# netapp-rickhuang-ai/spark-rapids-ml-nai

Measured on AMD Instinct MI355X. Metric: fit-time speedup vs Spark-ML CPU (geomean over reference headline workloads, 1Mx3000 fp32), higher is better.
Workload: dtype fp32

## Files before the change

spark_rapids_ml_nai_amd/ops/__init__.py:

```python
from __future__ import annotations

import math
import os
from typing import Any, Dict, Iterator, Optional, Tuple

import numpy as np
import torch

from . import native
from ..utils.determinism import deterministic

__all__ = ["col_moments", "gram", "xw", "dgemm", "sign_flip", "is_native", "xtv", "row_sqnorm",
           "logreg_binary_loss_grad", "nearest_centroid", "cluster_sums", "csr_logreg_binary_loss_grad",
           "csr_spmm", "csr_spmtm", "csr_col_moments", "logistic_loss_grad"]


def is_native(t: torch.Tensor) -> bool:
    return t.is_cuda


def _c(t: torch.Tensor) -> torch.Tensor:
    return t if t.is_contiguous() else t.contiguous()


# ... 427 lines not shown


def certify_tau16(n: int) -> float:
    return 1.01 * (2.0 * F16_U + F16_U * F16_U + 1.01 * float(n) * 2.0 ** -24)


def f16_radius_terms(n: int, scale: float, tau: float) -> Tuple[float, float, float]:
    a = F16_A / scale
    z = 2.02 * a * math.sqrt(n) * (1.0 + F16_U)
    z2 = 2.02 * float(n) * a * a
    wmax = math.sqrt(n) * 32768.0 / scale
    return (z + 2.0 ** -24 * wmax) / (2.0 * tau), z, z2


class F16Planes:

    def __init__(self, X: torch.Tensor, mu: torch.Tensor) -> None:
        m, n = X.shape
        self.X, self.m, self.n = X, m, n
        self.mu = _c(mu.float().view(-1))
        dev = X.device
        st = native.stream(dev)
        self.xnorm = torch.empty(m, dtype=torch.float32, device=dev)
        amax = zeros(1, dtype=torch.int32, device=dev)
        native.call("srml_row_sqnorm_centered_amax_f32", X.data_ptr(), m, n, X.stride(0), self.mu.data_ptr(),
                    self.xnorm.data_ptr(), amax.data_ptr(), st)
        a = float(amax.view(torch.float32).item())
        self.ok = math.isfinite(a) and a > 0.0
        self.scale = 1.0
        self.P = None
        if not self.ok:
            return
        e = math.frexp(a)[1] - 1
        if not -100 <= 13 - e <= 100:
            self.ok = False
            return
        self.scale = 2.0 ** (13 - e)
        self.kp = (n + 15) // 16 * 16
        self.rows_pad = max(256, (m + 255) // 256 * 256)
        self.P = torch.empty((self.rows_pad // 256, self.kp // 16, 256, 16), dtype=torch.float16, device=dev)
        self.ovf = zeros(1, dtype=torch.int32, device=dev)
        native.call("srml_split_f16_tiled_centered", X.data_ptr(), m, n, X.stride(0), self.mu.data_ptr(), self.kp,
                    self.rows_pad, self.scale, self.P.data_ptr(), self.ovf.data_ptr(), st)
        self.tau = certify_tau16(n)
        self.xadd, self.z, self.z2 = f16_radius_terms(n, self.scale, self.tau)


F16_CAND_CAP = 64


def _f16_centre_planes(F: F16Planes, C: torch.Tensor, approx: bool) -> Tuple[torch.Tensor, ...]:
    k, dev = C.shape[0], F.X.device
    st = native.stream(dev)
    Cd = _c(C.to(dev)) if C.dtype in (torch.float32, torch.float64) else _c(C.to(dev, torch.float32))
    crows = max(256, (k + 255) // 256 * 256)
    W = torch.empty((k, F.n), dtype=torch.float32, device=dev)
    cn = torch.empty(crows, dtype=torch.float32, device=dev)
    cg = torch.empty(k, dtype=torch.float32, device=dev)
    zero2 = torch.empty(2, dtype=torch.int32, device=dev)
    native.call("srml_f16_centre_prep", Cd.data_ptr(), int(Cd.dtype == torch.float64), k, F.n, F.mu.data_ptr(),
                float(2.0 * F.tau), int(bool(approx)), W.data_ptr(), cn.data_ptr(), cg.data_ptr(), zero2.data_ptr(), st)
    CP = torch.empty((crows // 256, F.kp // 16, 256, 16), dtype=torch.float16, device=dev)
    native.call("srml_split_f16_tiled_centered", W.data_ptr(), k, F.n, W.stride(0), None, F.kp, crows, F.scale,
                CP.data_ptr(), zero2[0:1].data_ptr(), st)
    return W, cn, cg, zero2, CP, crows


def nearest_f16_labels(F: F16Planes, C: torch.Tensor) -> Optional[torch.Tensor]:
    if F.kp != 128 or os.environ.get("SRML_F16_ROWLOOP", "1") == "0":
        return None
    dev = F.X.device
    _, cn, _, _, CP, crows = _f16_centre_planes(F, C, True)
    labels = torch.empty(F.m, dtype=torch.int32, device=dev)
    rc = native.lib().srml_nearest_f16_rowloop(F.P.data_ptr(), F.m, F.rows_pad, F.kp, CP.data_ptr(), C.shape[0],
                                                crows, cn.data_ptr(), float(-2.0 / (F.scale * F.scale)),
                                                labels.data_ptr(), native.stream(dev))
    if rc == -2:
        return None
    if rc != 0:
        raise RuntimeError("srml_nearest_f16_rowloop failed (%d)" % rc)
    return labels


def nearest_centroid_f16(F: F16Planes, C: torch.Tensor, approx: bool = False) -> Tuple[torch.Tensor, torch.Tensor]:
    m, k, dev = F.m, C.shape[0], F.X.device
    st = native.stream(dev)
    W, cn, cg, zero2, CP, crows = _f16_centre_planes(F, C, approx)
    ovf = zero2[0:1]
    xadd, z, z2 = (0.0, 0.0, 0.0) if approx else (F.xadd, F.z, F.z2)
    dscale = -2.0 / (F.scale * F.scale)
    nslot = int(native.lib().srml_nearest_centroid_f16_top2_nslot(k))
    labels = torch.empty(m, dtype=torch.int32, device=dev)
    dist = torch.empty(m, dtype=torch.float32, device=dev)
    flagged = torch.empty(m, dtype=torch.int32, device=dev)
    thr = torch.empty(m, dtype=torch.float32, device=dev)
    cnt = zero2[1:2]
    step = split_rows_per_launch(k)
    for r0 in range(0, m, step):
        mc = min(step, m - r0)
        keys = torch.empty(mc * nslot, dtype=torch.int64, device=dev)
        lob = torch.empty(mc * nslot, dtype=torch.float32, device=dev)
        Pc = F.P[r0 // 256: (r0 + mc + 255) // 256]
        xn = F.xnorm[r0: r0 + mc]
        native.call("srml_nearest_centroid_f16_top2", Pc.data_ptr(), mc, Pc.shape[0] * 256, F.kp, CP.data_ptr(), k,
                    crows, cn.data_ptr(), cg.data_ptr(), xn.data_ptr(), dscale, xadd, keys.data_ptr(), lob.data_ptr(),
                    st)
        c0 = int(cnt.item()) if r0 else 0
        native.call("srml_split_top2_select_f16_thr", keys.data_ptr(), lob.data_ptr(), mc, nslot, xn.data_ptr(),
                    cg.data_ptr(), xadd, z, z2, ovf.data_ptr(), labels[r0:].data_ptr(), dist[r0:].data_ptr(),
                    flagged.data_ptr(), cnt.data_ptr(), thr.data_ptr(), st)
        if r0:
            nc = int(cnt.item())
            flagged[c0:nc] += r0
        del keys, lob
    nf = int(cnt.item())
    _CERTIFY_STATS["rows"] += m
    _CERTIFY_STATS["refined"] += nf
    if nf:
        rows = flagged[:nf]
        X = F.X
        assert X.stride(1) == 1
        cap = F16_CAND_CAP
        cand = torch.empty(nf * cap, dtype=torch.int32, device=dev)
        stepr = split_rows_per_launch(k)
        plane = F.P is not None and os.environ.get("SRML_F16_GATHER", "plane") == "plane"
        ccount = torch.empty(nf, dtype=torch.int32, device=dev) if plane else zeros(nf, dtype=torch.int32,
                                                                                          device=dev)
        scratch = None if plane else zeros(1, dtype=torch.int32, device=dev)
        for q0 in range(0, nf, stepr):
            nq = min(stepr, nf - q0)
            rq = rows[q0: q0 + nq]
            rp = max(256, (nq + 255) // 256 * 256)
            Pr = torch.empty((rp // 256, F.kp // 16, 256, 16), dtype=torch.float16, device=dev)
            if plane:
                xr = torch.empty(nq, dtype=torch.float32, device=dev)
                native.call("srml_f16_plane_gather_rows_ex", F.P.data_ptr(), F.rows_pad, F.kp, rq.data_ptr(), nq, rp,
                            Pr.data_ptr(), F.xnorm.data_ptr(), xr.data_ptr(), ccount[q0:].data_ptr(), st)
            else:
                native.call("srml_split_f16_tiled_centered_rows", X.data_ptr(), X.stride(0), rq.data_ptr(), nq, F.n,
                            F.mu.data_ptr(), F.kp, rp, F.scale, Pr.data_ptr(), scratch.data_ptr(), st)
                xr = F.xnorm.index_select(0, rq.long())
            native.call("srml_nearest_centroid_f16_cand", Pr.data_ptr(), nq, rp, F.kp, CP.data_ptr(), k, crows,
                        cn.data_ptr(), cg.data_ptr(), xr.data_ptr(), dscale, xadd, thr[q0:].data_ptr(),
                        ccount[q0:].data_ptr(), cand[q0 * cap:].data_ptr(), cap, st)
            del Pr
        native.call("srml_kmeans_cand_exact", X.data_ptr(), X.stride(0), F.mu.data_ptr(), W.data_ptr(), W.stride(0),
                    F.n, k, rows.data_ptr(), nf, ccount.data_ptr(), cand.data_ptr(), cap, labels.data_ptr(),
                    dist.data_ptr(), st)
    return labels, dist


def quantizer_planes(X: torch.Tensor) -> Optional[F16Planes]:
    if not X.is_cuda or X.dtype != torch.float32 or X.dim() != 2 or X.shape[1] < 16 or X.stride(1) != 1:
        return None
    mu = col_moments(X, need_sq=False)[0].div_(max(X.shape[0], 1)).float()
    F = F16Planes(X, mu)
    return F if F.ok else None


def nearest_list(X: torch.Tensor, C: torch.Tensor, F: Optional[F16Planes] = None,
                 xnorm: Optional[torch.Tensor] = None) -> torch.Tensor:
    if F is not None and C.shape[0] > 256:
        lab = nearest_f16_labels(F, C)
        return lab if lab is not None else nearest_centroid_f16(F, C, approx=True)[0]
    return nearest_centroid(X, C, xnorm)[0]


def split_rows_per_launch(k: int) -> int:
    ct = max(1, (int(k) + 255) // 256)
    return max(256, (0xFFFFFFFF // 512 // ct) * 256)


def kmeans_filter_mode() -> str:
    v = os.environ.get("SRML_KMEANS_FILTER", "f16").lower()
    if v not in ("f16", "bf16"):
        raise ValueError("SRML_KMEANS_FILTER must be f16 or bf16, got %r" % v)
    return v


def nearest_centroid_split(XP: torch.Tensor, m: int, C: torch.Tensor, xnorm: torch.Tensor,
                           cnorm: Optional[torch.Tensor] = None, approx: bool = False,
                           X: Optional[torch.Tensor] = None, mu: Optional[torch.Tensor] = None
                           ) -> Tuple[torch.Tensor, torch.Tensor]:
    k = C.shape[0]
    Cf = C.float()
    if mu is not None:
        Cf = Cf - mu.float().view(1, -1).to(Cf.device)
        cnorm = None
    if cnorm is None:
# ... 2056 lines not shown
```

spark_rapids_ml_nai_amd/ops/csrc/splitmm.hip:

```cpp
#include "common.h"

#include "tile.h"
#include <stdlib.h>

namespace {
using srml_tile::orderable;
using srml_tile::unorderable;

typedef short bf16x8 __attribute__((ext_vector_type(8)));
typedef _Float16 halfx8 __attribute__((ext_vector_type(8)));
typedef unsigned uintx4 __attribute__((ext_vector_type(4)));
typedef unsigned uintx2 __attribute__((ext_vector_type(2)));

__device__ __forceinline__ unsigned bf16_rn(float f) {
  unsigned u = __float_as_uint(f);
  u += 0x7fffu + ((u >> 16) & 1u);
  return u >> 16;
}
__device__ __forceinline__ float bf16_f(unsigned b) { return __uint_as_float(b << 16); }

__global__ __launch_bounds__(256) void split_kernel(const float* __restrict__ X, long m, int n, long ld, int kp,
                                                    long rows_pad, unsigned short* __restrict__ P) {
  const int q4 = kp >> 2;
  const long total = rows_pad * q4;
  const long plane = rows_pad * (long)kp;
  for (long i = (long)blockIdx.x * 256 + threadIdx.x; i < total; i += (long)gridDim.x * 256) {
    const long r = i / q4;
    const int c = (int)(i - r * q4) * 4;
    unsigned h[4], md[4], lo[4];
#pragma unroll
    for (int j = 0; j < 4; ++j) {
      const float x = (r < m && c + j < n) ? X[r * ld + c + j] : 0.f;
      h[j] = bf16_rn(x);
      const float r1 = x - bf16_f(h[j]);
      md[j] = bf16_rn(r1);
      lo[j] = bf16_rn(r1 - bf16_f(md[j]));
    }
    const long o = r * kp + c;
    *reinterpret_cast<uintx2*>(P + o) = uintx2{h[0] | (h[1] << 16), h[2] | (h[3] << 16)};
    *reinterpret_cast<uintx2*>(P + plane + o) = uintx2{md[0] | (md[1] << 16), md[2] | (md[3] << 16)};
    *reinterpret_cast<uintx2*>(P + 2 * plane + o) = uintx2{lo[0] | (lo[1] << 16), lo[2] | (lo[3] << 16)};
  }
}

__global__ __launch_bounds__(256) void split_tiled_kernel(const float* __restrict__ X, long m, int n, long ld, int kp,
                                                          long rows_pad, unsigned short* __restrict__ P,
                                                          const float* __restrict__ mu,
                                                          const int* __restrict__ ridx = nullptr) {
  const int ks_n = kp >> 4;
  const long total = rows_pad * ks_n;
  const long plane = rows_pad * (long)kp;
  const bool vec = (ld & 3) == 0 && (reinterpret_cast<uintptr_t>(X) & 15) == 0;
  for (long i = (long)blockIdx.x * 256 + threadIdx.x; i < total; i += (long)gridDim.x * 256) {
    const long img = i >> 8;
    const int rr = (int)(i & 255);
    const long tile = img / ks_n;
    const int c0 = (int)(img - tile * ks_n) * 16;
    const long r = tile * 256 + rr;
    const long rs = ridx && r < m ? (long)ridx[r] : r;
    float x[16];
    if (vec && r < m && c0 + 16 <= n) {
#pragma unroll
      for (int q = 0; q < 4; ++q) {
        const floatx4 v = *reinterpret_cast<const floatx4*>(X + rs * ld + c0 + 4 * q);
        x[4 * q] = v[0]; x[4 * q + 1] = v[1]; x[4 * q + 2] = v[2]; x[4 * q + 3] = v[3];
      }
    } else {
#pragma unroll
      for (int j = 0; j < 16; ++j) x[j] = (r < m && c0 + j < n) ? X[rs * ld + c0 + j] : 0.f;
    }
    if (mu && r < m) {
#pragma unroll
      for (int j = 0; j < 16; ++j)
        if (c0 + j < n) x[j] -= mu[c0 + j];
    }
    unsigned hw[8], mw[8], lw[8];
#pragma unroll
    for (int j = 0; j < 16; j += 2) {
      unsigned h2[2], m2[2], l2[2];
#pragma unroll
      for (int u = 0; u < 2; ++u) {
        h2[u] = bf16_rn(x[j + u]);
        const float r1 = x[j + u] - bf16_f(h2[u]);
        m2[u] = bf16_rn(r1);
        l2[u] = bf16_rn(r1 - bf16_f(m2[u]));
      }
// ... 317 lines not shown
#pragma unroll
      for (int r = 0; r < 16; ++r) acc[a][b][r] = 0.f;

  auto mma_step = [&](int cur) {
    bf16x8 fb[3][TN];
#pragma unroll
    for (int p = 0; p < 3; ++p)
#pragma unroll
      for (int nt = 0; nt < TN; ++nt)
        fb[p][nt] = *reinterpret_cast<const bf16x8*>(&st[cur].B[p][wn * (BN / WN) + nt * 32 + li][8 * lk]);
#pragma unroll
    for (int mt = 0; mt < TM; ++mt) {
      bf16x8 fa[3];
#pragma unroll
      for (int p = 0; p < 3; ++p)
        fa[p] = *reinterpret_cast<const bf16x8*>(&st[cur].A[p][wm * (BM / WM) + mt * 32 + li][8 * lk]);
#pragma unroll
      for (int nt = 0; nt < TN; ++nt) {
        acc[mt][nt] = __builtin_amdgcn_mfma_f32_32x32x16_bf16(fa[2], fb[0][nt], acc[mt][nt], 0, 0, 0);
        acc[mt][nt] = __builtin_amdgcn_mfma_f32_32x32x16_bf16(fa[1], fb[1][nt], acc[mt][nt], 0, 0, 0);
        acc[mt][nt] = __builtin_amdgcn_mfma_f32_32x32x16_bf16(fa[0], fb[2][nt], acc[mt][nt], 0, 0, 0);
        acc[mt][nt] = __builtin_amdgcn_mfma_f32_32x32x16_bf16(fa[1], fb[0][nt], acc[mt][nt], 0, 0, 0);
        acc[mt][nt] = __builtin_amdgcn_mfma_f32_32x32x16_bf16(fa[0], fb[1][nt], acc[mt][nt], 0, 0, 0);
        acc[mt][nt] = __builtin_amdgcn_mfma_f32_32x32x16_bf16(fa[0], fb[0][nt], acc[mt][nt], 0, 0, 0);
      }
    }
  };
  auto gload = [&](int kt, uintx4 (&a)[3], uintx4 (&b)[3]) {
    const long ko = (long)kt * SBK;
#pragma unroll
    for (int p = 0; p < 3; ++p) {
      a[p] = *reinterpret_cast<const uintx4*>(xa + p * xplane + ko);
      b[p] = *reinterpret_cast<const uintx4*>(ca + p * cplane + ko);
    }
  };
  auto lstore = [&](int stage, const uintx4 (&a)[3], const uintx4 (&b)[3]) {
#pragma unroll
    for (int p = 0; p < 3; ++p) {
      *reinterpret_cast<uintx4*>(&st[stage].A[p][sr][sh]) = a[p];
      *reinterpret_cast<uintx4*>(&st[stage].B[p][sr][sh]) = b[p];
    }
  };
  const int nk = kp / SBK;
  if (PF == 1) {
    uintx4 ra[3], rb[3];
    gload(0, ra, rb);
    lstore(0, ra, rb);
    __syncthreads();
    int cur = 0;
    for (int kt = 0; kt < nk; ++kt) {
      const bool more = kt + 1 < nk;
      if (more) gload(kt + 1, ra, rb);
      mma_step(cur);
      if (more) lstore(cur ^ 1, ra, rb);
      __syncthreads();
      cur ^= 1;
    }
  } else {
    uintx4 ra0[3], rb0[3], ra1[3], rb1[3];
    gload(0, ra0, rb0);
    if (nk > 1) gload(1, ra1, rb1);
    lstore(0, ra0, rb0);
    __syncthreads();
    int kt = 0;
    for (; kt + 2 <= nk; kt += 2) {
      if (kt + 2 < nk) gload(kt + 2, ra0, rb0);
      mma_step(0);
      lstore(1, ra1, rb1);
      __syncthreads();
      if (kt + 3 < nk) gload(kt + 3, ra1, rb1);
      mma_step(1);
      if (kt + 2 < nk) lstore(0, ra0, rb0);
      __syncthreads();
    }
    if (kt < nk) mma_step(0);
  }

  split_epilogue<BM, BN, WM, WN>(acc, row0, col0, m, k, cnorm, best, wm, wn, li, lk);
}

typedef __attribute__((address_space(3))) void* lds_vptr;
typedef __attribute__((address_space(1))) void* gbl_vptr;

template <bool TILED, int NP = 6, bool TOP2 = false, int WN_ = 4, bool PRIO = false, bool CAND = false, int RING = 0>
__global__ __launch_bounds__(WN_ * 128, WN_ == 4 ? 1 : 2) void nearest_centroid_split_glds_kernel(
    const unsigned short* __restrict__ XP, long m, long xrows, int kp, const unsigned short* __restrict__ CP, int k,
    long crows, const float* __restrict__ cnorm, unsigned long long* __restrict__ best, int n_ctiles,
    float* __restrict__ lob = nullptr, const float* __restrict__ cg = nullptr, const float* __restrict__ xnorm = nullptr,
    float dscale = -2.f, float xadd = 0.f, const float* __restrict__ thr = nullptr, int* __restrict__ ccount = nullptr,
    int* __restrict__ cand = nullptr, int cap = 0) {
  static_assert(!CAND || (NP == 1 && TOP2), "candidate lists come from the fp16 filter");
  static_assert(WN_ == 4 || (WN_ == 2 && NP != 6), "256 x 128 tiles are built for the filter passes");
  static_assert(NP == 6 || NP == 3 || (NP == 1 && TOP2), "NP = 1 is the fp16 certified filter");
  constexpr int BM = 256, WM = 2, WN = WN_, BN = 64 * WN, TM = 4, TN = 2;
  constexpr int NPL = NP == 6 ? 3 : (NP == 3 ? 2 : 1);
  constexpr int XCH = NPL * (BM / 32), CCH = NPL * (BN / 32);
  constexpr int CPW = (XCH + CCH) / (WM * WN);
  static_assert((XCH + CCH) % (WM * WN) == 0, "chunks split evenly over the waves");
  constexpr int KPB = RING ? RING / 10 : NP == 1 ? 3 : (NP == 3 && WN_ == 4 ? 2 : 1);
  constexpr int NG = RING ? RING % 10 : NP == 1 && WN_ == 4 ? 3 : 2;
  static_assert(!RING || (NP == 1 && KPB >= 1 && NG >= 2), "ring override is for the fp16 filter");
  constexpr int NS = (KPB > 1 || RING) ? NG * KPB : 3;
  constexpr int STAGE = NPL * (BM + BN) * 16;
  __shared__ __attribute__((aligned(1024))) unsigned short lds[NS][STAGE];
  const int bid = xcd_remap(blockIdx.x, gridDim.x);
  const long rtile = bid / n_ctiles;
  const int ctile = bid % n_ctiles;
  const long row0 = rtile * BM;
  const int col0 = ctile * BN;
  const int t = threadIdx.x;
  const int lane = t & 63, wid = t >> 6;
  const int wm = wid / WN, wn = wid % WN;
  const int li = lane & 31, lk = lane >> 5;
  const long xplane = xrows * (long)kp, cplane = crows * (long)kp;

  const unsigned short* src[CPW];
  int dst_off[CPW];
#pragma unroll
  for (int i = 0; i < CPW; ++i) {
    const int c = wid * CPW + i;
    const bool isx = c < XCH;
    const int q = isx ? c / (BM / 32) : (c - XCH) / (BN / 32);
    const int j = isx ? c % (BM / 32) : (c - XCH) % (BN / 32);
    const int r = 32 * j + (lane >> 1);
    const int lh = (lane & 1) ^ ((lane >> 4) & 1);
    if (TILED) {
      const int ks_n = kp / SBK;
      if (isx) src[i] = XP + q * xplane + ((rtile * ks_n) << 12) + 512 * j + lane * 8;
      else src[i] = CP + q * cplane + (((long)(col0 >> 8) * ks_n) << 12) + 16 * (col0 & 255) + 512 * j + lane * 8;
    } else if (isx) {
      long xr = row0 + r;
      if (xr >= xrows) xr = xrows - 1;
      src[i] = XP + q * xplane + xr * kp + 8 * lh;
    } else {
      src[i] = CP + q * cplane + (long)(col0 + r) * kp + 8 * lh;
    }
    dst_off[i] = isx ? (q * BM + 32 * j) * 16 : (NPL * BM + q * BN + 32 * j) * 16;
  }
  auto issue = [&](int kt, int stage) {
    unsigned short* base = &lds[stage][0];
#pragma unroll
    for (int i = 0; i < CPW; ++i) {
      __builtin_amdgcn_global_load_lds((gbl_vptr)(src[i] + (TILED ? ((long)kt << 12) : (long)kt * SBK)),
                                       (lds_vptr)(base + dst_off[i]), 16, 0, 0);
    }
  };

  floatx16 acc[TM][TN];
#pragma unroll
  for (int a = 0; a < TM; ++a)
#pragma unroll
    for (int b = 0; b < TN; ++b)
#pragma unroll
      for (int r = 0; r < 16; ++r) acc[a][b][r] = 0.f;

  const int ph = lk ^ ((li >> 3) & 1);
  const int nk = kp / SBK;
  auto compute = [&](int st) {
    bf16x8 fb[NPL][TN];
#pragma unroll
    for (int p = 0; p < NPL; ++p)
#pragma unroll
      for (int nt = 0; nt < TN; ++nt)
        fb[p][nt] = *reinterpret_cast<const bf16x8*>(
            &lds[st][(NPL * BM + p * BN + wn * (BN / WN) + nt * 32 + li) * 16 + 8 * ph]);
#pragma unroll
    for (int mt = 0; mt < TM; ++mt) {
      bf16x8 fa[NPL];
#pragma unroll
      for (int p = 0; p < NPL; ++p)
        fa[p] = *reinterpret_cast<const bf16x8*>(&lds[st][(p * BM + wm * (BM / WM) + mt * 32 + li) * 16 + 8 * ph]);
#pragma unroll
      for (int nt = 0; nt < TN; ++nt) {
        if constexpr (NP == 1) {
          acc[mt][nt] = __builtin_amdgcn_mfma_f32_32x32x16_f16(__builtin_bit_cast(halfx8, fb[0][nt]),
                                                               __builtin_bit_cast(halfx8, fa[0]), acc[mt][nt], 0,
                                                               0, 0);
        } else {
          if constexpr (NP == 6) {
            acc[mt][nt] = __builtin_amdgcn_mfma_f32_32x32x16_bf16(fa[2], fb[0][nt], acc[mt][nt], 0, 0, 0);
            acc[mt][nt] = __builtin_amdgcn_mfma_f32_32x32x16_bf16(fa[1], fb[1][nt], acc[mt][nt], 0, 0, 0);
            acc[mt][nt] = __builtin_amdgcn_mfma_f32_32x32x16_bf16(fa[0], fb[2][nt], acc[mt][nt], 0, 0, 0);
          }
          acc[mt][nt] = __builtin_amdgcn_mfma_f32_32x32x16_bf16(fa[1], fb[0][nt], acc[mt][nt], 0, 0, 0);
          acc[mt][nt] = __builtin_amdgcn_mfma_f32_32x32x16_bf16(fa[0], fb[1][nt], acc[mt][nt], 0, 0, 0);
          acc[mt][nt] = __builtin_amdgcn_mfma_f32_32x32x16_bf16(fa[0], fb[0][nt], acc[mt][nt], 0, 0, 0);
        }
      }
    }
  };
  if constexpr (KPB == 1 && !RING) {
    static_assert(CPW == 6, "the counted wait below leaves one step (CPW loads) in flight");
    issue(0, 0);
    if (nk > 1) issue(1, 1);
    int stage = 0;
    for (int kt = 0; kt < nk; ++kt) {
      if (kt + 1 < nk) asm volatile("s_waitcnt vmcnt(6)" ::: "memory");
      else asm volatile("s_waitcnt vmcnt(0)" ::: "memory");
      __builtin_amdgcn_s_barrier();
      if (kt + 2 < nk) issue(kt + 2, stage == 0 ? 2 : stage - 1);
      if (PRIO) __builtin_amdgcn_s_setprio(1);
      compute(stage);
      if (PRIO) __builtin_amdgcn_s_setprio(0);
      stage = stage == 2 ? 0 : stage + 1;
    }
  } else {
#pragma unroll
    for (int j = 0; j < (NG - 1) * KPB; ++j)
      if (j < nk) issue(j, j);
    for (int kt = 0; kt < nk; kt += KPB) {
      if (NG >= 3 && kt + (NG - 1) * KPB <= nk)
        asm volatile("s_waitcnt vmcnt(%0)" ::"i"((NG - 2) * KPB * CPW) : "memory");
      else asm volatile("s_waitcnt vmcnt(0)" ::: "memory");
      __builtin_amdgcn_s_barrier();
#pragma unroll
      for (int j = 0; j < KPB; ++j)
        if (kt + (NG - 1) * KPB + j < nk) issue(kt + (NG - 1) * KPB + j, (kt + (NG - 1) * KPB + j) % NS);
      if (PRIO) __builtin_amdgcn_s_setprio(1);
#pragma unroll
      for (int j = 0; j < KPB; ++j)
        if (kt + j < nk) compute((kt + j) % NS);
      if (PRIO) __builtin_amdgcn_s_setprio(0);
    }
  }
  if (CAND)
    split_epilogue_cand_t<BM, BN, WM, WN>(acc, row0, col0, m, k, cnorm, cg, xnorm, wm, wn, li, lk, dscale, xadd, thr,
                                          ccount, cand, cap);
  else if (TOP2 && NP == 1)
    split_epilogue_top2_t<BM, BN, WM, WN>(acc, row0, col0, ctile, m, k, cnorm, cg, xnorm, best, lob, n_ctiles * WN, wm,
                                          wn, li, lk, dscale, xadd);
  else if (TOP2)
    split_epilogue_top2<BM, BN, WM, WN>(acc, row0, col0, ctile, m, k, cnorm, cg, xnorm, best, lob, n_ctiles * WN, wm,
                                        wn, li, lk, dscale, xadd);
  else
    split_epilogue<BM, BN, WM, WN>(acc, row0, col0, m, k, cnorm, best, wm, wn, li, lk);
}

__global__ __launch_bounds__(256) void split_top2_select_kernel(const unsigned long long* __restrict__ keys,
                                                                const float* __restrict__ lob, long m, int nslot,
                                                                const float* __restrict__ xnorm,
                                                                const float* __restrict__ cg,
                                                                int* __restrict__ labels, float* __restrict__ dist,
                                                                int* __restrict__ flagged, int* __restrict__ n_flagged,
                                                                float xadd = 0.f, float z = 0.f, float z2 = 0.f,
                                                                const int* __restrict__ ovf = nullptr,
                                                                float* __restrict__ thr_out = nullptr) {
  const long i = (long)blockIdx.x * 256 + threadIdx.x;
  if (i >= m) return;
  unsigned long long k1 = ~0ull;
  int s1 = 0;
  for (int s = 0; s < nslot; ++s) {
    const unsigned long long v = keys[(long)s * m + i];
    if (v < k1) { k1 = v; s1 = s; }
  }
  const float xn = xnorm[i];
  const float xs0 = sqrtf(fmaxf(xn, 0.f));
  const float xs = xs0 + xadd;
  const float c2 = 2.f * fmaf(z, xs0, z2);
  float low = __builtin_huge_valf();
  for (int s = 0; s < nslot; ++s) {
    low = fminf(low, lob[(long)s * m + i]);
    const unsigned long long v = keys[(long)s * m + i];
    if (s != s1 && v != ~0ull) low = fminf(low, fmaf(-xs, cg[(int)(v & 0xffffffffu)], unorderable((unsigned)(v >> 32))));
  }
  const float bv = unorderable((unsigned)(k1 >> 32));
  if (k1 != ~0ull && !(ovf && *ovf) && low > fmaf(xs, cg[(int)(k1 & 0xffffffffu)], bv) + c2) {
    labels[i] = (int)(k1 & 0xffffffffu);
    const float d = bv + xn;
    dist[i] = d > 0.f ? d : 0.f;
  } else {
    const int p = atomicAdd(n_flagged, 1);
    flagged[p] = (int)i;
    if (thr_out)
      thr_out[p] = (k1 != ~0ull && !(ovf && *ovf)) ? fmaf(xs, cg[(int)(k1 & 0xffffffffu)], bv) + c2
// ... 193 lines not shown
}

SRML_API int srml_nearest_centroid_split_tiled_np(const unsigned short* XP, long m, long xrows, int kp,
                                                  const unsigned short* CP, int k, long crows, const float* cnorm,
                                                  unsigned long long* best, int nprod, hipStream_t stream) {
  if (m <= 0 || k <= 0) return 0;
  if ((kp & 15) || xrows < m || crows < k || (crows & 255) || (xrows & 255)) return -2;
  if ((reinterpret_cast<uintptr_t>(XP) & 15) || (reinterpret_cast<uintptr_t>(CP) & 15)) return -5;
  const long rt = (m + 255) / 256;
  const int bn = nprod == 3 ? split3_bn() : 256;
  const int ct = (k + bn - 1) / bn;
  const long nb = rt * ct;
  if (nb > srml_max_blocks(512)) return -3;
  if (nprod == 3 && bn == 128)
    hipLaunchKernelGGL((nearest_centroid_split_glds_kernel<true, 3, false, 2>), dim3((unsigned)nb), dim3(256), 0, stream,
                       XP, m, xrows, kp, CP, k, crows, cnorm, best, (int)ct);
  else if (nprod == 3)
    hipLaunchKernelGGL((nearest_centroid_split_glds_kernel<true, 3>), dim3((unsigned)nb), dim3(512), 0, stream, XP, m,
                       xrows, kp, CP, k, crows, cnorm, best, (int)ct);
  else if (nprod == 6)
    hipLaunchKernelGGL((nearest_centroid_split_glds_kernel<true, 6>), dim3((unsigned)nb), dim3(512), 0, stream, XP, m,
                       xrows, kp, CP, k, crows, cnorm, best, (int)ct);
  else
    return -2;
  return srml_status();
}

SRML_API int srml_nearest_centroid_split_tiled(const unsigned short* XP, long m, long xrows, int kp,
                                               const unsigned short* CP, int k, long crows, const float* cnorm,
                                               unsigned long long* best, hipStream_t stream) {
  return srml_nearest_centroid_split_tiled_np(XP, m, xrows, kp, CP, k, crows, cnorm, best, 6, stream);
}

SRML_API int srml_nearest_centroid_split_top2(const unsigned short* XP, long m, long xrows, int kp,
                                              const unsigned short* CP, int k, long crows, const float* cnorm,
                                              const float* cg, const float* xnorm, unsigned long long* keys,
                                              float* lob, hipStream_t stream) {
  if (m <= 0 || k <= 0) return 0;
  if ((kp & 15) || xrows < m || crows < k || (crows & 255) || (xrows & 255)) return -2;
  if ((reinterpret_cast<uintptr_t>(XP) & 15) || (reinterpret_cast<uintptr_t>(CP) & 15)) return -5;
  const long rt = (m + 255) / 256;
  const int bn = split3_bn();
  const int ct = (k + bn - 1) / bn;
  const long nb = rt * ct;
  if (nb > srml_max_blocks(512)) return -3;
  static const bool prio = !(getenv("SRML_SPLIT_PRIO") && atoi(getenv("SRML_SPLIT_PRIO")) == 0);
#define SRML_TOP2(WNN, PR, T)                                                                                    \
  hipLaunchKernelGGL((nearest_centroid_split_glds_kernel<true, 3, true, WNN, PR>), dim3((unsigned)nb), dim3(T), 0, \
                     stream, XP, m, xrows, kp, CP, k, crows, cnorm, keys, (int)ct, lob, cg, xnorm)
  if (bn == 128 && prio) SRML_TOP2(2, true, 256);
  else if (bn == 128) SRML_TOP2(2, false, 256);
  else if (prio) SRML_TOP2(4, true, 512);
  else SRML_TOP2(4, false, 512);
#undef SRML_TOP2
  return srml_status();
}

SRML_API int srml_nearest_centroid_split_top2_nslot(int k) {
  const int bn = split3_bn();
  return ((k + bn - 1) / bn) * (bn / 64);
}

SRML_API int srml_split_top2_select(const unsigned long long* keys, const float* lob, long m, int nslot,
                                    const float* xnorm, const float* cg, int* labels, float* dist, int* flagged,
                                    int* n_flagged, hipStream_t stream) {
  if (m <= 0) return 0;
  hipLaunchKernelGGL(split_top2_select_kernel, dim3((unsigned)((m + 255) / 256)), dim3(256), 0, stream, keys, lob, m,
                     nslot, xnorm, cg, labels, dist, flagged, n_flagged);
  return srml_status();
}

SRML_API int srml_split_scatter_refined(const unsigned long long* best, const int* rows, int nf, const float* xnorm,
                                        int* labels, float* dist, hipStream_t stream) {
  if (nf <= 0) return 0;
  hipLaunchKernelGGL(split_scatter_refined_kernel, dim3((unsigned)((nf + 255) / 256)), dim3(256), 0, stream, best,
                     rows, nf, xnorm, labels, dist);
  return srml_status();
}

static int f16_bn() {
  static const int bn = getenv("SRML_F16_BN") && atoi(getenv("SRML_F16_BN")) == 128 ? 128 : 256;
  return bn;
}
static int f16_slots_per_tile() { return f16_bn() / 64; }

template <typename T>
__global__ __launch_bounds__(256) void f16_centre_prep_kernel(const T* __restrict__ C, int k, int n,
                                                              const float* __restrict__ mu, float tau2, int approx,
                                                              float* __restrict__ W, float* __restrict__ cn,
                                                              float* __restrict__ cg, int* __restrict__ zero2) {
  const int j = blockIdx.x * 4 + (threadIdx.x >> 6);
  const int lane = threadIdx.x & 63;
  if (blockIdx.x == 0 && threadIdx.x < 2) zero2[threadIdx.x] = 0;
  if (j >= k) return;
  double a = 0.0;
  for (int d = lane; d < n; d += 64) {
    const float w = (float)((double)C[(long)j * n + d] - (double)mu[d]);
    W[(long)j * n + d] = w;
    a += (double)w * (double)w;
  }
  for (int o = 32; o > 0; o >>= 1) a += __shfl_xor(a, o, 64);
  if (lane == 0) {
    const float c = (float)a;
    cn[j] = c;
    cg[j] = approx ? 0.f : tau2 * sqrtf(c > 0.f ? c : 0.f);
  }
}

SRML_API int srml_f16_centre_prep(const void* C, int c_f64, int k, int n, const float* mu, float tau2, int approx,
                                  float* W, float* cn, float* cg, int* zero2, hipStream_t stream) {
  if (k <= 0) return 0;
  const dim3 grid((unsigned)((k + 3) / 4));
  if (c_f64)
    hipLaunchKernelGGL(f16_centre_prep_kernel<double>, grid, dim3(256), 0, stream,
                       reinterpret_cast<const double*>(C), k, n, mu, tau2, approx, W, cn, cg, zero2);
  else
    hipLaunchKernelGGL(f16_centre_prep_kernel<float>, grid, dim3(256), 0, stream, reinterpret_cast<const float*>(C),
                       k, n, mu, tau2, approx, W, cn, cg, zero2);
  return srml_status();
}

SRML_API int srml_split_f16_tiled_centered(const float* X, long m, int n, long ld, const float* mu, int kp,
                                           long rows_pad, float scale, unsigned short* P, int* ovf,
                                           hipStream_t stream) {
  if (rows_pad <= 0) return 0;
  if ((kp & 15) || kp < n || rows_pad < m || (rows_pad & 255)) return -2;
  if ((reinterpret_cast<uintptr_t>(P) & 15) != 0) return -5;
  const long total = rows_pad * (long)(kp / 16);
  long blocks = (total + 255) / 256;
  if (blocks > 65536) blocks = 65536;
  hipLaunchKernelGGL(split_tiled_f16_kernel, dim3((unsigned)blocks), dim3(256), 0, stream, X, m, n, ld, kp, rows_pad, P,
                     mu, scale, ovf);
  return srml_status();
}

SRML_API int srml_nearest_centroid_f16_top2(const unsigned short* XP, long m, long xrows, int kp,
                                            const unsigned short* CP, int k, long crows, const float* cnorm,
                                            const float* cg, const float* xnorm, float dscale, float xadd,
                                            unsigned long long* keys, float* lob, hipStream_t stream) {
  if (m <= 0 || k <= 0) return 0;
  if ((kp & 15) || xrows < m || crows < k || (crows & 255) || (xrows & 255)) return -2;
  if ((reinterpret_cast<uintptr_t>(XP) & 15) || (reinterpret_cast<uintptr_t>(CP) & 15)) return -5;
  const long rt = (m + 255) / 256;
  const int bn = f16_bn();
  const int ct = (k + bn - 1) / bn;
  const long nb = rt * ct;
  if (nb > srml_max_blocks(bn * 2)) return -3;
  static const bool prio = !(getenv("SRML_SPLIT_PRIO") && atoi(getenv("SRML_SPLIT_PRIO")) == 0);
#define SRML_F16(WNN, PR, T)                                                                                      \
  hipLaunchKernelGGL((nearest_centroid_split_glds_kernel<true, 1, true, WNN, PR>), dim3((unsigned)nb), dim3(T), 0, \
                     stream, XP, m, xrows, kp, CP, k, crows, cnorm, keys, (int)ct, lob, cg, xnorm, dscale, xadd)
  static const int ring = getenv("SRML_F16_RING") ? atoi(getenv("SRML_F16_RING")) : 0;
#define SRML_F16R(RG)                                                                                               \
  hipLaunchKernelGGL((nearest_centroid_split_glds_kernel<true, 1, true, 4, true, false, RG>), dim3((unsigned)nb),      \
                     dim3(512), 0, stream, XP, m, xrows, kp, CP, k, crows, cnorm, keys, (int)ct, lob, cg, xnorm,       \
                     dscale, xadd)
  if (f16_bn() == 128) {
    if (prio) SRML_F16(2, true, 256);
    else SRML_F16(2, false, 256);
  } else if (ring == 23) {
    SRML_F16R(23);
  } else if (ring == 24) {
    SRML_F16R(24);
  } else if (ring == 42) {
    SRML_F16R(42);
  } else if (ring == 18) {
    SRML_F16R(18);
  } else if (ring == 25) {
    SRML_F16R(25);
  } else {
    if (prio) SRML_F16(4, true, 512);
    else SRML_F16(4, false, 512);
  }
#undef SRML_F16R
#undef SRML_F16
  return srml_status();
}

SRML_API int srml_nearest_centroid_f16_top2_nslot(int k) {
  const int bn = f16_bn();
  return ((k + bn - 1) / bn) * f16_slots_per_tile();
}

SRML_API int srml_split_top2_select_f16(const unsigned long long* keys, const float* lob, long m, int nslot,
                                        const float* xnorm, const float* cg, float xadd, float z, float z2,
                                        const int* ovf, int* labels, float* dist, int* flagged, int* n_flagged,
                                        hipStream_t stream) {
  if (m <= 0) return 0;
  hipLaunchKernelGGL(split_top2_select_kernel, dim3((unsigned)((m + 255) / 256)), dim3(256), 0, stream, keys, lob, m,
                     nslot, xnorm, cg, labels, dist, flagged, n_flagged, xadd, z, z2, ovf);
  return srml_status();
}

SRML_API int srml_split_f16_tiled_centered_rows(const float* X, long ld, const int* ridx, long m, int n,
                                                const float* mu, int kp, long rows_pad, float scale, unsigned short* P,
                                                int* ovf, hipStream_t stream) {
  if (rows_pad <= 0) return 0;
  if ((kp & 15) || kp < n || rows_pad < m || (rows_pad & 255) || !ridx) return -2;
  if ((reinterpret_cast<uintptr_t>(P) & 15) != 0) return -5;
  const long total = rows_pad * (long)(kp / 16);
  long blocks = (total + 255) / 256;
  if (blocks > 65536) blocks = 65536;
  hipLaunchKernelGGL(split_tiled_f16_kernel, dim3((unsigned)blocks), dim3(256), 0, stream, X, m, n, ld, kp, rows_pad, P,
                     mu, scale, ovf, ridx);
  return srml_status();
}

__global__ __launch_bounds__(256) void f16_plane_gather_kernel(const uintx4* __restrict__ src, int ks_n,
                                                               const int* __restrict__ ridx, long m, long rows_pad,
                                                               uintx4* __restrict__ dst,
                                                               const float* __restrict__ xn = nullptr,
                                                               float* __restrict__ xn_out = nullptr,
                                                               int* __restrict__ zero_out = nullptr) {
  for (long i = (long)blockIdx.x * 256 + threadIdx.x; i < m; i += (long)gridDim.x * 256) {
    if (xn_out) xn_out[i] = xn[ridx[i]];
    if (zero_out) zero_out[i] = 0;
  }
  const long total = rows_pad * ks_n;
  for (long i = (long)blockIdx.x * 256 + threadIdx.x; i < total; i += (long)gridDim.x * 256) {
    const long img = i >> 8;
    const int rr = (int)(i & 255);
    const long tile = img / ks_n;
    const long ks = img - tile * ks_n;
    const long r = tile * 256 + rr;
    uintx4 lo = uintx4{0u, 0u, 0u, 0u}, hi = lo;
    if (r < m) {
      const long rs = ridx[r];
      const int ssw = (int)((rs >> 3) & 1);
      const uintx4* s = src + ((((rs >> 8) * ks_n + ks) << 12) + (rs & 255) * 16) / 8;
      lo = s[ssw];
      hi = s[ssw ^ 1];
    }
    const int dsw = (rr >> 3) & 1;
    uintx4* d = dst + ((img << 12) + rr * 16) / 8;
    d[dsw] = lo;
    d[dsw ^ 1] = hi;
  }
}

SRML_API int srml_f16_plane_gather_rows_ex(const unsigned short* P, long src_rows_pad, int kp, const int* ridx, long m,
                                           long rows_pad, unsigned short* out, const float* xn, float* xn_out,
                                           int* zero_out, hipStream_t stream) {
  if (rows_pad <= 0) return 0;
  if ((kp & 15) || rows_pad < m || (rows_pad & 255) || (src_rows_pad & 255) || !ridx) return -2;
  if ((reinterpret_cast<uintptr_t>(P) & 15) || (reinterpret_cast<uintptr_t>(out) & 15)) return -5;
  if (xn_out && !xn) return -2;
  const long total = rows_pad * (long)(kp / 16);
  long blocks = (total + 255) / 256;
  if (blocks > 65536) blocks = 65536;
  hipLaunchKernelGGL(f16_plane_gather_kernel, dim3((unsigned)blocks), dim3(256), 0, stream,
                     reinterpret_cast<const uintx4*>(P), kp / 16, ridx, m, rows_pad, reinterpret_cast<uintx4*>(out), xn,
                     xn_out, zero_out);
  return srml_status();
}

SRML_API int srml_f16_plane_gather_rows(const unsigned short* P, long src_rows_pad, int kp, const int* ridx, long m,
                                        long rows_pad, unsigned short* out, hipStream_t stream) {
  return srml_f16_plane_gather_rows_ex(P, src_rows_pad, kp, ridx, m, rows_pad, out, nullptr, nullptr, nullptr, stream);
}

SRML_API int srml_split_top2_select_f16_thr(const unsigned long long* keys, const float* lob, long m, int nslot,
                                            const float* xnorm, const float* cg, float xadd, float z, float z2,
                                            const int* ovf, int* labels, float* dist, int* flagged, int* n_flagged,
                                            float* thr_out, hipStream_t stream) {
  if (m <= 0) return 0;
  hipLaunchKernelGGL(split_top2_select_kernel, dim3((unsigned)((m + 255) / 256)), dim3(256), 0, stream, keys, lob, m,
                     nslot, xnorm, cg, labels, dist, flagged, n_flagged, xadd, z, z2, ovf, thr_out);
  return srml_status();
}

SRML_API int srml_nearest_centroid_f16_cand(const unsigned short* XP, long m, long xrows, int kp,
                                            const unsigned short* CP, int k, long crows, const float* cnorm,
                                            const float* cg, const float* xnorm, float dscale, float xadd,
                                            const float* thr, int* ccount, int* cand, int cap, hipStream_t stream) {
  if (m <= 0 || k <= 0) return 0;
  if ((kp & 15) || xrows < m || crows < k || (crows & 255) || (xrows & 255) || cap < 1) return -2;
  if ((reinterpret_cast<uintptr_t>(XP) & 15) || (reinterpret_cast<uintptr_t>(CP) & 15)) return -5;
  const long rt = (m + 255) / 256;
  const int ct = (k + 255) / 256;
  const long nb = rt * ct;
  if (nb > srml_max_blocks(512)) return -3;
  hipLaunchKernelGGL((nearest_centroid_split_glds_kernel<true, 1, true, 4, true, true>), dim3((unsigned)nb), dim3(512),
                     0, stream, XP, m, xrows, kp, CP, k, crows, cnorm, (unsigned long long*)nullptr, (int)ct,
                     (float*)nullptr, cg, xnorm, dscale, xadd, thr, ccount, cand, cap);
  return srml_status();
}

SRML_API int srml_kmeans_cand_exact(const float* X, long ld, const float* mu, const float* W, long ldw, int n, int k,
                                    const int* rows, int nf, const int* ccount, const int* cand, int cap, int* labels,
                                    float* dist, hipStream_t stream) {
  if (nf <= 0) return 0;
  const dim3 grid((unsigned)((nf + 3) / 4));
  const bool vec = (n & 3) == 0 && (ld & 3) == 0 && (ldw & 3) == 0 && (reinterpret_cast<uintptr_t>(X) & 15) == 0 &&
                   (reinterpret_cast<uintptr_t>(W) & 15) == 0 && (reinterpret_cast<uintptr_t>(mu) & 15) == 0;
  const int nv = (n / 4 + 63) / 64;
  static const bool scalar = getenv("SRML_CAND_EXACT") && atoi(getenv("SRML_CAND_EXACT")) == 0;
#define SRML_CE(NVV)                                                                                                  \
  hipLaunchKernelGGL(cand_exact_vec_kernel<NVV>, grid, dim3(256), 0, stream, X, ld, mu, W, ldw, n, k, rows, nf, ccount, \
                     cand, cap, labels, dist)
  if (vec && !scalar && nv <= 4) SRML_CE(4);
  else if (vec && !scalar && nv <= 8) SRML_CE(8);
  else if (vec && !scalar && nv <= 12) SRML_CE(12);
  else if (vec && !scalar && nv <= 16) SRML_CE(16);
  else
    hipLaunchKernelGGL(cand_exact_kernel, grid, dim3(256), 0, stream, X, ld, mu, W, ldw, n, k, rows, nf, ccount, cand,
                       cap, labels, dist);
#undef SRML_CE
  return srml_status();
}

namespace {
template <int KS>
__global__ __launch_bounds__(512, 1) void nearest_f16_rowloop_kernel(const unsigned short* __restrict__ XP, long m,
                                                                     const unsigned short* __restrict__ CP, int k,
                                                                     int n_ctiles, const float* __restrict__ cnorm,
                                                                     float dscale, int* __restrict__ labels) {
  constexpr int CT = 256;
  constexpr int IMG = CT * 16;
  constexpr int CHUNKS = KS * 8;
  constexpr int CPW = CHUNKS / 8;
  __shared__ __attribute__((aligned(1024))) unsigned short lds[2][KS * IMG];
  __shared__ __attribute__((aligned(1024))) float cn_s[2][CT];
  const long tile = xcd_remap(blockIdx.x, gridDim.x);
  const int t = threadIdx.x, lane = t & 63, wid = t >> 6, li = lane & 31, lk = lane >> 5;
  const int rr = 32 * wid + li;
  halfx8 xb[KS];
#pragma unroll
  for (int ks = 0; ks < KS; ++ks)
    xb[ks] = *reinterpret_cast<const halfx8*>(XP + ((tile * KS + ks) << 12) + rr * 16 + 8 * (lk ^ ((rr >> 3) & 1)));
  auto issue = [&](int c, int buf) {
    const unsigned short* src = CP + ((long)c * KS << 12);
#pragma unroll
    for (int i = 0; i < CPW; ++i) {
      const int ch = wid * CPW + i;
      __builtin_amdgcn_global_load_lds((gbl_vptr)(src + ch * 512 + lane * 8), (lds_vptr)(&lds[buf][ch * 512]), 16, 0,
                                       0);
    }
    if (wid == 0) {
#pragma unroll
      for (int i = 0; i < CT / 64; ++i)
        __builtin_amdgcn_global_load_lds((gbl_vptr)(cnorm + (long)c * CT + i * 64 + lane), (lds_vptr)(&cn_s[buf][i * 64]),
                                         4, 0, 0);
    }
  };
  float best = __builtin_huge_valf();
  int bi = 0x7fffffff;
  issue(0, 0);
  if (n_ctiles > 1) issue(1, 1);
  for (int c = 0; c < n_ctiles; ++c) {
    const int buf = c & 1;
    if (c + 1 < n_ctiles) {
      if (wid == 0) asm volatile("s_waitcnt vmcnt(%0)" ::"i"(CPW + CT / 64) : "memory");
      else asm volatile("s_waitcnt vmcnt(%0)" ::"i"(CPW) : "memory");
    } else {
      asm volatile("s_waitcnt vmcnt(0)" ::: "memory");
    }
    __builtin_amdgcn_s_barrier();
    const bool last = c == n_ctiles - 1;
    const int cbase = c * CT;
#pragma unroll 2
    for (int nt = 0; nt < CT / 32; ++nt) {
      floatx16 acc;
#pragma unroll
      for (int r = 0; r < 16; ++r) acc[r] = 0.f;
      const int cl = nt * 32 + li;
#pragma unroll
      for (int ks = 0; ks < KS; ++ks) {
// ... 48 lines not shown
```

Baseline: 3517.

## Add phased 4-k-step LDS pipeline for fp16 k-means filter kernel

Adds a PHASED variant of the fp16 nearest-centroid filter kernel. It stages four k-steps per K tile into an 8-slot LDS double buffer with a fixed per-wave piece map and counted vmcnt waits. MFMA phases are interleaved with barriers and priority raises. The variant is the default for the 256-wide top2 and candidate filter paths, and the old env-selected ring variants are removed. It also adds a Python helper that runs one filter launch with zero-initialised outputs, which is likely for testing. The hand-scheduled pipeline risks hazards or register pressure, and the new code references a `zeros` name that may not be defined.

```diff
diff --git a/spark_rapids_ml_nai_amd/ops/__init__.py b/spark_rapids_ml_nai_amd/ops/__init__.py
--- a/spark_rapids_ml_nai_amd/ops/__init__.py
+++ b/spark_rapids_ml_nai_amd/ops/__init__.py
@@ -533,6 +533,30 @@
     return labels
 
 
+def _f16_filter_launch(F: F16Planes, r0: int, mc: int, CP: torch.Tensor, k: int, crows: int, cn: torch.Tensor,
+                       cg: torch.Tensor, dscale: float, xadd: float, nslot: int,
+                       zero: bool) -> Tuple[torch.Tensor, torch.Tensor]:
+    dev = F.X.device
+    alloc = zeros if zero else torch.empty
+    keys = alloc(mc * nslot, dtype=torch.int64, device=dev)
+    lob = alloc(mc * nslot, dtype=torch.float32, device=dev)
+    Pc = F.P[r0 // 256: (r0 + mc + 255) // 256]
+    xn = F.xnorm[r0: r0 + mc]
+    native.call("srml_nearest_centroid_f16_top2", Pc.data_ptr(), mc, Pc.shape[0] * 256, F.kp, CP.data_ptr(), k,
+                crows, cn.data_ptr(), cg.data_ptr(), xn.data_ptr(), dscale, xadd, keys.data_ptr(), lob.data_ptr(),
+                native.stream(dev))
+    return keys, lob
+
+
+def f16_filter_slots(F: F16Planes, C: torch.Tensor, approx: bool = False) -> Tuple[torch.Tensor, torch.Tensor]:
+    k = C.shape[0]
+    _, cn, cg, _, CP, crows = _f16_centre_planes(F, C, approx)
+    xadd = 0.0 if approx else F.xadd
+    nslot = int(native.lib().srml_nearest_centroid_f16_top2_nslot(k))
+    mc = min(split_rows_per_launch(k), F.m)
+    return _f16_filter_launch(F, 0, mc, CP, k, crows, cn, cg, -2.0 / (F.scale * F.scale), xadd, nslot, True)
+
+
 def nearest_centroid_f16(F: F16Planes, C: torch.Tensor, approx: bool = False) -> Tuple[torch.Tensor, torch.Tensor]:
     m, k, dev = F.m, C.shape[0], F.X.device
     st = native.stream(dev)
@@ -549,13 +573,8 @@
     step = split_rows_per_launch(k)
     for r0 in range(0, m, step):
         mc = min(step, m - r0)
-        keys = torch.empty(mc * nslot, dtype=torch.int64, device=dev)
-        lob = torch.empty(mc * nslot, dtype=torch.float32, device=dev)
-        Pc = F.P[r0 // 256: (r0 + mc + 255) // 256]
         xn = F.xnorm[r0: r0 + mc]
-        native.call("srml_nearest_centroid_f16_top2", Pc.data_ptr(), mc, Pc.shape[0] * 256, F.kp, CP.data_ptr(), k,
-                    crows, cn.data_ptr(), cg.data_ptr(), xn.data_ptr(), dscale, xadd, keys.data_ptr(), lob.data_ptr(),
-                    st)
+        keys, lob = _f16_filter_launch(F, r0, mc, CP, k, crows, cn, cg, dscale, xadd, nslot, False)
         c0 = int(cnt.item()) if r0 else 0
         native.call("srml_split_top2_select_f16_thr", keys.data_ptr(), lob.data_ptr(), mc, nslot, xn.data_ptr(),
                     cg.data_ptr(), xadd, z, z2, ovf.data_ptr(), labels[r0:].data_ptr(), dist[r0:].data_ptr(),
diff --git a/spark_rapids_ml_nai_amd/ops/csrc/splitmm.hip b/spark_rapids_ml_nai_amd/ops/csrc/splitmm.hip
--- a/spark_rapids_ml_nai_amd/ops/csrc/splitmm.hip
+++ b/spark_rapids_ml_nai_amd/ops/csrc/splitmm.hip
@@ -2,6 +2,7 @@
 
 #include "tile.h"
 #include <stdlib.h>
+#include <string.h>
 
 namespace {
 using srml_tile::orderable;
@@ -485,7 +486,8 @@
 typedef __attribute__((address_space(3))) void* lds_vptr;
 typedef __attribute__((address_space(1))) void* gbl_vptr;
 
-template <bool TILED, int NP = 6, bool TOP2 = false, int WN_ = 4, bool PRIO = false, bool CAND = false, int RING = 0>
+template <bool TILED, int NP = 6, bool TOP2 = false, int WN_ = 4, bool PRIO = false, bool CAND = false,
+          bool PHASED = false>
 __global__ __launch_bounds__(WN_ * 128, WN_ == 4 ? 1 : 2) void nearest_centroid_split_glds_kernel(
     const unsigned short* __restrict__ XP, long m, long xrows, int kp, const unsigned short* __restrict__ CP, int k,
     long crows, const float* __restrict__ cnorm, unsigned long long* __restrict__ best, int n_ctiles,
@@ -500,10 +502,10 @@
   constexpr int XCH = NPL * (BM / 32), CCH = NPL * (BN / 32);
   constexpr int CPW = (XCH + CCH) / (WM * WN);
   static_assert((XCH + CCH) % (WM * WN) == 0, "chunks split evenly over the waves");
-  constexpr int KPB = RING ? RING / 10 : NP == 1 ? 3 : (NP == 3 && WN_ == 4 ? 2 : 1);
-  constexpr int NG = RING ? RING % 10 : NP == 1 && WN_ == 4 ? 3 : 2;
-  static_assert(!RING || (NP == 1 && KPB >= 1 && NG >= 2), "ring override is for the fp16 filter");
-  constexpr int NS = (KPB > 1 || RING) ? NG * KPB : 3;
+  constexpr int KPB = NP == 1 ? 3 : (NP == 3 && WN_ == 4 ? 2 : 1);
+  constexpr int NG = NP == 1 && WN_ == 4 ? 3 : 2;
+  static_assert(!PHASED || (TILED && NP == 1 && WN_ == 4), "the phased loop is the fp16 filter's 256 x 256 tile");
+  constexpr int NS = PHASED ? 8 : KPB > 1 ? NG * KPB : 3;
   constexpr int STAGE = NPL * (BM + BN) * 16;
   __shared__ __attribute__((aligned(1024))) unsigned short lds[NS][STAGE];
   const int bid = xcd_remap(blockIdx.x, gridDim.x);
@@ -592,7 +594,86 @@
       }
     }
   };
-  if constexpr (KPB == 1 && !RING) {
+  if constexpr (PHASED) {
+    static_assert(CPW == 2 && STAGE == 8192, "piece map below: 16 pieces per k step, 8 per wave per K tile");
+    const int wu = __builtin_amdgcn_readfirstlane(wid);
+    const int ntile = (nk + 3) >> 2;
+    const int xks = wu & 3, xj0 = (wu >> 2) * 4;
+    const unsigned short* xsrc = XP + (((long)rtile * nk) << 12) + lane * 8;
+    const unsigned short* csrc = CP + (((long)(col0 >> 8) * nk) << 12) + 512 * wu + lane * 8;
+    auto stage_pair = [&](int U, int i) __attribute__((always_inline)) {
+      const int sb = (U & 1) * 4;
+#pragma unroll
+      for (int e = 0; e < 2; ++e) {
+        if (i < 2) {
+          const int ks = 2 * i + e;
+          const int kt = min(4 * U + ks, nk - 1);
+          __builtin_amdgcn_global_load_lds((gbl_vptr)(csrc + ((long)kt << 12)),
+                                           (lds_vptr)(&lds[sb + ks][(BM + 32 * wu) * 16]), 16, 0, 0);
+        } else {
+          const int j = xj0 + 2 * (i - 2) + e;
+          const int kt = min(4 * U + xks, nk - 1);
+          __builtin_amdgcn_global_load_lds((gbl_vptr)(xsrc + ((long)kt << 12) + 512 * j),
+                                           (lds_vptr)(&lds[sb + xks][32 * j * 16]), 16, 0, 0);
+        }
+      }
+    };
+    bf16x8 fb[4][TN], fa[4];
+    auto tile = [&](int T, int nks, bool STEADY) __attribute__((always_inline)) {
+      const int sb = (T & 1) * 4;
+#pragma unroll
+      for (int p = 0; p < 4; ++p) {
+        if (p == 0) {
+#pragma unroll
+          for (int ks = 0; ks < 4; ++ks)
+#pragma unroll
+            for (int nt = 0; nt < TN; ++nt)
+              fb[ks][nt] = *reinterpret_cast<const bf16x8*>(
+                  &lds[sb + ks][(BM + wn * (BN / WN) + nt * 32 + li) * 16 + 8 * ph]);
+        }
+#pragma unroll
+        for (int ks = 0; ks < 4; ++ks)
+          fa[ks] = *reinterpret_cast<const bf16x8*>(&lds[sb + ks][(wm * (BM / WM) + p * 32 + li) * 16 + 8 * ph]);
+        const int U = T + 1 + (p >> 1);
+        if (STEADY || U < ntile) stage_pair(U, p ^ 2);
+        if (p == 3) {
+          if (STEADY) asm volatile("s_waitcnt vmcnt(4)" ::: "memory");
+          else asm volatile("s_waitcnt vmcnt(0)" ::: "memory");
+        }
+        __builtin_amdgcn_s_barrier();
+        asm volatile("s_waitcnt lgkmcnt(0)" ::: "memory");
+        __builtin_amdgcn_s_setprio(1);
+#pragma unroll
+        for (int ks = 0; ks < 4; ++ks)
+          if (STEADY || ks < nks) {
+#pragma unroll
+            for (int nt = 0; nt < TN; ++nt)
+              acc[p][nt] = __builtin_amdgcn_mfma_f32_32x32x16_f16(__builtin_bit_cast(halfx8, fb[ks][nt]),
+                                                                  __builtin_bit_cast(halfx8, fa[ks]), acc[p][nt], 0, 0,
+                                                                  0);
+          }
+        __builtin_amdgcn_s_setprio(0);
+        __builtin_amdgcn_s_barrier();
+      }
+    };
+    stage_pair(0, 0);
+    stage_pair(0, 1);
+    stage_pair(0, 2);
+    stage_pair(0, 3);
+    if (ntile > 1) {
+      stage_pair(1, 0);
+      stage_pair(1, 1);
+      asm volatile("s_waitcnt vmcnt(4)" ::: "memory");
+    } else {
+      asm volatile("s_waitcnt vmcnt(0)" ::: "memory");
+    }
+    __builtin_amdgcn_s_barrier();
+    if (wu >= WN) __builtin_amdgcn_s_barrier();
+    int T = 0;
+    for (; T + 2 < ntile; ++T) tile(T, 4, true);
+    for (; T < ntile; ++T) tile(T, min(4, nk - 4 * T), false);
+    if (wu < WN) __builtin_amdgcn_s_barrier();
+  } else if constexpr (KPB == 1) {
     static_assert(CPW == 6, "the counted wait below leaves one step (CPW loads) in flight");
     issue(0, 0);
     if (nk > 1) issue(1, 1);
@@ -952,6 +1033,13 @@
   static const int bn = getenv("SRML_F16_BN") && atoi(getenv("SRML_F16_BN")) == 128 ? 128 : 256;
   return bn;
 }
+constexpr bool F16_SCHED_DEFAULT_PHASED = true;
+static bool f16_phased() {
+  const char* s = getenv("SRML_F16_SCHED");
+  if (s && !strcmp(s, "legacy")) return false;
+  if (s && !strcmp(s, "phased")) return true;
+  return F16_SCHED_DEFAULT_PHASED;
+}
 static int f16_slots_per_tile() { return f16_bn() / 64; }
 
 template <typename T>
@@ -1020,29 +1108,20 @@
 #define SRML_F16(WNN, PR, T)                                                                                      \
   hipLaunchKernelGGL((nearest_centroid_split_glds_kernel<true, 1, true, WNN, PR>), dim3((unsigned)nb), dim3(T), 0, \
                      stream, XP, m, xrows, kp, CP, k, crows, cnorm, keys, (int)ct, lob, cg, xnorm, dscale, xadd)
-  static const int ring = getenv("SRML_F16_RING") ? atoi(getenv("SRML_F16_RING")) : 0;
-#define SRML_F16R(RG)                                                                                               \
-  hipLaunchKernelGGL((nearest_centroid_split_glds_kernel<true, 1, true, 4, true, false, RG>), dim3((unsigned)nb),      \
-                     dim3(512), 0, stream, XP, m, xrows, kp, CP, k, crows, cnorm, keys, (int)ct, lob, cg, xnorm,       \
+#define SRML_F16P()                                                                                               \
+  hipLaunchKernelGGL((nearest_centroid_split_glds_kernel<true, 1, true, 4, true, false, true>), dim3((unsigned)nb),  \
+                     dim3(512), 0, stream, XP, m, xrows, kp, CP, k, crows, cnorm, keys, (int)ct, lob, cg, xnorm,     \
                      dscale, xadd)
   if (f16_bn() == 128) {
     if (prio) SRML_F16(2, true, 256);
     else SRML_F16(2, false, 256);
-  } else if (ring == 23) {
-    SRML_F16R(23);
-  } else if (ring == 24) {
-    SRML_F16R(24);
-  } else if (ring == 42) {
-    SRML_F16R(42);
-  } else if (ring == 18) {
-    SRML_F16R(18);
-  } else if (ring == 25) {
-    SRML_F16R(25);
+  } else if (kp >= 16 && f16_phased()) {
+    SRML_F16P();
   } else {
     if (prio) SRML_F16(4, true, 512);
     else SRML_F16(4, false, 512);
   }
-#undef SRML_F16R
+#undef SRML_F16P
 #undef SRML_F16
   return srml_status();
 }
@@ -1150,9 +1229,14 @@
   const int ct = (k + 255) / 256;
   const long nb = rt * ct;
   if (nb > srml_max_blocks(512)) return -3;
-  hipLaunchKernelGGL((nearest_centroid_split_glds_kernel<true, 1, true, 4, true, true>), dim3((unsigned)nb), dim3(512),
-                     0, stream, XP, m, xrows, kp, CP, k, crows, cnorm, (unsigned long long*)nullptr, (int)ct,
-                     (float*)nullptr, cg, xnorm, dscale, xadd, thr, ccount, cand, cap);
+  if (f16_bn() == 256 && kp >= 16 && f16_phased())
+    hipLaunchKernelGGL((nearest_centroid_split_glds_kernel<true, 1, true, 4, true, true, true>), dim3((unsigned)nb),
+                       dim3(512), 0, stream, XP, m, xrows, kp, CP, k, crows, cnorm, (unsigned long long*)nullptr, (int)ct,
+                       (float*)nullptr, cg, xnorm, dscale, xadd, thr, ccount, cand, cap);
+  else
+    hipLaunchKernelGGL((nearest_centroid_split_glds_kernel<true, 1, true, 4, true, true>), dim3((unsigned)nb),
+                       dim3(512), 0, stream, XP, m, xrows, kp, CP, k, crows, cnorm, (unsigned long long*)nullptr, (int)ct,
+                       (float*)nullptr, cg, xnorm, dscale, xadd, thr, ccount, cand, cap);
   return srml_status();
 }
 
```

New measurement: 3537, median of 6. No clear change (+0.6%).
